# alpha-davidson/TensorBNN

Measured on AMD Instinct MI355X. Metric: leapfrog steps/sec (whole node), higher is better.
Workload: dtype f32

## Files before the change

tensorbnn_amd/csrc/fused_ops.hpp:

```cpp
#pragma once
#include <hip/hip_runtime.h>
#include "common.hpp"
#include "wide_api.hpp"

#define TBNN_JIT_ABI 7
enum { TBNN_FAMILY_NARROW = 1, TBNN_FAMILY_WIDE = 2 };

struct FusedOps {
    int abi;
    int family;
    int nl, dims[TBNN_MAX_LAYERS + 1];
    int hact, lact, lik;
    char name[128];
    int img_floats;
    void (*image_map)(int* map );
    int (*grid)(long n);
    int (*launch)(int grid, hipStream_t st, const NetDev* nd, const float* qimg, const float* eta, const float* X,
                  const float* Y, long n, float* slabs, int pitch, double* pstat, int nchains, ChainStride cs);
    int (*nforward)(int gx, int nets, hipStream_t st, const float* qimgs, long img_stride, const float* X, long n, float* fouts,
                    long out_stride);
    int traj_max_rows;
    int (*traj)(int nchains, hipStream_t st, const NetDev* nd, const float* qimg, long img_stride, const float* eta, const float* X, const float* Y, long n,
                float* q, float* p, float* g, float* gd, const int* imgmap, double* pstat, int nstat, float eps, int L, const StepCtl* ctl);
    void (*plan)(long n, WidePlan* plan);
    int (*wlaunch)(const WidePlan* plan, hipStream_t st, const NetDev* nd, const float* qimg, const float* eta,
                   const float* X, const float* Y, long n, float* store, float* slabA, float* slabB, double* pstat, float* out);
    int (*wforward)(hipStream_t st, const NetDev* nd, const float* qimg, const float* X, long n, float* fout);
};

static inline bool fused_ops_match(const FusedOps& o, const NetDev& nd, bool weighted = false) {
    if (o.nl != nd.nl || o.lik != (shape_lik(nd.lik) | (weighted ? SHAPE_LIK_WEIGHTED : 0))) return false;
    for (int l = 0; l < nd.nl; ++l) {
        if (nd.in[l] != o.dims[l] || nd.out[l] != o.dims[l + 1]) return false;
        if (nd.act[l] != (l == nd.nl - 1 ? o.lact : ((o.hact & TBNN_ACT_PACKED) ? (o.hact >> (3 * l)) & 7 : o.hact))) return false;
    }
    return true;
}

template <class S>
static inline void fused_ops_shape(FusedOps* o, const char* prefix, const char* name = nullptr) {
    o->abi = TBNN_JIT_ABI;
    o->nl = S::NL;
    for (int i = 0; i <= S::NL; ++i) o->dims[i] = S::D[i];
    o->hact = S::HCODE; o->lact = S::LACT; o->lik = S::LIK;
    if (name) { snprintf(o->name, sizeof(o->name), "%s", name); return; }
    static const char* an[] = {"none", "relu", "tanh", "sigmoid", "exp", "elu", "?", "?"};
    int k = snprintf(o->name, sizeof(o->name), "%s<", prefix);
    if (S::HCODE & TBNN_ACT_PACKED) {
// ... 7 lines not shown
```

tensorbnn_amd/csrc/jit_mid.hpp:

```cpp
#pragma once
#include "kernels_mid.hpp"
#include "fused_ops.hpp"

template <class S>
struct JitMid {
    static int grid(long n) { return mid_grid(n); }
    static int launch(int g, hipStream_t st, const NetDev* nd, const float* qimg, const float* eta, const float* X, const float* Y,
                      long n, float* slabs, int pitch, double* pstat, int nchains, ChainStride cs) {
        return mid_launch_t<S>(g, st, *nd, qimg, eta, X, Y, n, slabs, pitch, pstat, nchains, cs);
    }
    static int nforward(int gx, int nets, hipStream_t st, const float* qimgs, long img_stride, const float* X, long n, float* fouts,
                        long out_stride) {
        return mid_forward_t<S>(gx, nets, st, qimgs, img_stride, X, n, fouts, out_stride);
    }
    static void image_map(int* map) { mid_image_map<S>(map); }
    static void fill(FusedOps* o, const char* name = nullptr) {
        fused_ops_shape<S>(o, "jit-mid", name);
        o->family = TBNN_FAMILY_NARROW;
        o->img_floats = MidCfg<S>::IMG_FLOATS;
        o->image_map = &image_map; o->grid = &grid; o->launch = &launch; o->nforward = &nforward;
        o->plan = nullptr; o->wlaunch = nullptr; o->wforward = nullptr;
    }
};
```

tensorbnn_amd/csrc/jit_narrow.hpp:

```cpp
#pragma once
#include "kernels_fast3.hpp"
#include "kernels_traj.hpp"
#include "fused_ops.hpp"

template <class S, bool F3>
struct JitNarrow {
    static int grid(long n) {
        const long ntiles = (n + 15) / 16, wgs = (ntiles + FAST_WAVES - 1) / FAST_WAVES;
        return (int)(wgs < 256 ? wgs : 256);
    }
    static int launch_stamped(int g, hipStream_t st, const NetDev* nd, const float* qimg, const float* eta, const float* X, const float* Y,
                              long n, float* slabs, int pitch, double* pstat, int nchains, ChainStride cs, unsigned long long* stamps) {
        if constexpr (F3)
            hipLaunchKernelGGL(k_fwd_bwd_fast3<S>, dim3(g, nchains), dim3(FAST_THREADS), 0, st, *nd, qimg, eta, X, Y, n, slabs, pitch, pstat,
                               stamps, cs);
        else
            hipLaunchKernelGGL(k_fwd_bwd_fast<S>, dim3(g, nchains), dim3(FAST_THREADS), 0, st, *nd, qimg, eta, X, Y, n, slabs, pitch, pstat,
                               stamps, cs);
        return hipGetLastError() == hipSuccess ? 0 : -1;
    }
    static int launch(int g, hipStream_t st, const NetDev* nd, const float* qimg, const float* eta, const float* X, const float* Y,
                      long n, float* slabs, int pitch, double* pstat, int nchains, ChainStride cs) {
        return launch_stamped(g, st, nd, qimg, eta, X, Y, n, slabs, pitch, pstat, nchains, cs, nullptr);
    }
    static int nforward(int gx, int nets, hipStream_t st, const float* qimgs, long img_stride, const float* X, long n, float* fouts,
                        long out_stride) {
        if constexpr (F3) {
            hipLaunchKernelGGL(k_forward_fast3<S>, dim3(gx, nets), dim3(FAST_THREADS), 0, st, qimgs, img_stride, X, n, fouts, out_stride);
            return hipGetLastError() == hipSuccess ? 0 : -1;
        } else {
            return -1;
        }
    }
    static constexpr int TRAJ_NW = (!F3 || S::WTD || TBNN_TRAJ_WAVES == 0) ? 0 : (TBNN_TRAJ_WAVES == 16 && TrajCfg<S, 16>::OK) ? 16 : (TrajCfg<S, 4>::OK ? 4 : 0);
    static int traj(int nchains, hipStream_t st, const NetDev* nd, const float* qimg, long img_stride, const float* eta, const float* X, const float* Y, long n,
                    float* q, float* p, float* g, float* gd, const int* imgmap, double* pstat, int nstat, float eps, int L, const StepCtl* ctl) {
        if constexpr (TRAJ_NW > 0) {
            hipLaunchKernelGGL((k_traj_fast3<S, TRAJ_NW>), dim3(1, nchains), dim3(64 * TRAJ_NW), 0, st, *nd, qimg, img_stride, eta, X, Y, n, q, p, g, gd, imgmap,
                               pstat, nstat, eps, L, ctl);
            return hipGetLastError() == hipSuccess ? 0 : -1;
        } else {
            return -1;
        }
    }
    static void image_map(int* map) { ImageMap<S, 0>::run(map); }
    static void fill(FusedOps* o, const char* name = nullptr) {
        fused_ops_shape<S>(o, F3 ? "jit-fast3" : "jit-fast", name);
        o->family = TBNN_FAMILY_NARROW;
        o->img_floats = FastCfg<S>::STATIC_FLOATS;
        o->image_map = &image_map; o->grid = &grid; o->launch = &launch;
        o->nforward = F3 ? &nforward : nullptr;
        o->plan = nullptr; o->wlaunch = nullptr; o->wforward = nullptr;
        o->traj = TRAJ_NW > 0 ? &traj : nullptr;
        o->traj_max_rows = TRAJ_NW == 16 ? TBNN_TRAJ_MAX_ROWS : TRAJ_NW == 4 ? TBNN_TRAJ_MAX_ROWS_4 : 0;
    }
};

#ifdef TBNN_TILE_STAMPS
extern "C" int tbnn_jit_tile_stamps(unsigned long long* out64) {
    return hipMemcpyFromSymbol(out64, HIP_SYMBOL(g_tile_stamps), 64 * sizeof(unsigned long long)) == hipSuccess ? 0 : -1;
}
#endif
```

tensorbnn_amd/csrc/jit_tall.hpp:

```cpp
#pragma once
#include "kernels_tall.hpp"
#include "fused_ops.hpp"

template <class S>
struct JitTall {
    static int grid(long n) { return tall_grid<S>(n); }
    static int launch(int g, hipStream_t st, const NetDev* nd, const float* qimg, const float* eta, const float* X, const float* Y,
                      long n, float* slabs, int pitch, double* pstat, int nchains, ChainStride cs) {
        return tall_launch_t<S>(g, st, *nd, qimg, eta, X, Y, n, slabs, pitch, pstat, nchains, cs);
    }
    static int nforward(int gx, int nets, hipStream_t st, const float* qimgs, long img_stride, const float* X, long n, float* fouts,
                        long out_stride) {
        return tall_forward_t<S>(gx, nets, st, qimgs, img_stride, X, n, fouts, out_stride);
    }
    static void image_map(int* map) { tall_image_map<S>(map); }
    static void fill(FusedOps* o, const char* prefix = "jit-tall") {
        fused_ops_shape<S>(o, prefix);
        o->family = TBNN_FAMILY_NARROW;
        o->img_floats = TallCfg<S, TallPick<S>::NW>::IMG_FLOATS;
        o->image_map = &image_map; o->grid = &grid; o->launch = &launch; o->nforward = &nforward;
        o->plan = nullptr; o->wlaunch = nullptr; o->wforward = nullptr;
    }
};
```

tensorbnn_amd/csrc/jit_wide.hpp:

```cpp
#pragma once
#include "wide_api.hpp"
#include "kernels_wide.hpp"
#include "fused_ops.hpp"

template <class S>
struct JitWide {
    static void plan(long n, WidePlan* p) { p->id = -2; wide_plan_t<S>(n, *p); }
    static int wlaunch(const WidePlan* p, hipStream_t st, const NetDev* nd, const float* qimg, const float* eta, const float* X,
                       const float* Y, long n, float* store, float* slabA, float* slabB, double* pstat, float* out) {
        return wide_launch_t<S>(*p, st, *nd, qimg, eta, X, Y, n, store, slabA, slabB, pstat, out);
    }
    static int wforward(hipStream_t st, const NetDev* nd, const float* qimg, const float* X, long n, float* fout) {
        return wide_forward_t<S>(st, *nd, qimg, X, n, fout);
    }
    static void image_map(int* map) { wide_image_map<S>(map); }
    static void fill(FusedOps* o, const char* name = nullptr) {
        fused_ops_shape<S>(o, WideCfg<S>::RESIDENT ? "jit-wide(resident)" : "jit-wide", name);
        o->family = TBNN_FAMILY_WIDE;
        o->img_floats = WideCfg<S>::IMG_FLOATS;
        o->image_map = &image_map; o->grid = nullptr; o->launch = nullptr;
        o->plan = &plan; o->wlaunch = &wlaunch;
        o->wforward = wide_forward_ok<S>() ? &wforward : nullptr;
        o->nforward = nullptr;
    }
};
```

tensorbnn_amd/csrc/kernels_fast3.hpp:

```cpp
#pragma once
#include <type_traits>
#include "kernels_fast.hpp"

template <int I, int N, class F>
__device__ __forceinline__ void sfor3(F&& f) {
    if constexpr (I < N) { f(std::integral_constant<int, I>{}); sfor3<I + 1, N>(f); }
}
template <class S>
struct F3Cfg : FastCfg<S> {
    using B = FastCfg<S>;
    static constexpr int NF(int l) { return (B::out(l) % 16 == 1 || B::out(l) % 16 == 2) ? B::out(l) % 16 : 0; }
    static constexpr int MTF(int l) { return NF(l) ? B::MT(l) - 1 : B::MT(l); }
    static constexpr int fslot(int l, int f) { return 16 * MTF(l) + 4 * f; }
    static constexpr int funit(int l, int f) { return 16 * MTF(l) + f; }
    static constexpr int NLM3 = MTF(B::NL - 1) == 0 ? B::NL - 1 : B::NL;
    static_assert(NLM3 == B::NLM, "fast3 expects the same MFMA/VALU split of the last layer as fast");
    static constexpr int dw_tiles_plain() { int o = 0; for (int m = 0; m < NLM3; ++m) o += MTF(m) * B::NT(m); return o; }
    static constexpr bool NCF(int l) {
        return dw_tiles_plain() <= 39 && l < NLM3 && B::NT(l) >= 2 && MTF(l) >= 1 && MTF(l) <= 4 && B::in(l) + 1 - 16 * (B::NT(l) - 1) <= 4;
    }
    static constexpr int NTF(int l) { return NCF(l) ? B::NT(l) - 1 : B::NT(l); }
    static constexpr int dwt3(int l) { return MTF(l) * NTF(l) + (NCF(l) ? 2 : 0); }
    static constexpr int dwoff3(int l) { int o = 0; for (int m = 0; m < l && m < NLM3; ++m) o += dwt3(m); return o; }
    static constexpr int dwfr3(int l) { return dwoff3(l) + MTF(l) * NTF(l); }
    static constexpr int DW3_TILES = dwoff3(B::NL);
    static constexpr int KIN(int l) { return l == 0 ? B::KS0 : 4 * B::MT(l - 1); }
    static constexpr bool FB(int l) { return NF(l) > 0 && MTF(l) > 0; }
    static constexpr int fpn(int l) { return NF(l) == 0 ? 0 : (FB(l) ? 2 * B::NT(l) : NF(l) * (KIN(l) + 1)); }
    static constexpr int fpoff(int l) { int o = 0; for (int m = 0; m < l; ++m) o += fpn(m); return o; }
    static constexpr int FP_REGS = fpoff(B::NL);
    static constexpr int maxNF() { int m = 0; for (int l = 0; l < B::NL; ++l) m = NF(l) > m ? NF(l) : m; return m; }
    static constexpr int EP3_WANT = DW3_TILES * FAST_WAVES * 256 <= 39936 ? DW3_TILES : (DW3_TILES < 16 ? DW3_TILES : 16);
    static constexpr int PR = 16 + TBNN_PPAD;
    static constexpr int aoff3(int l) { int o = 0; for (int m = 0; m < l && m < NLM3; ++m) o += 16 * B::NT(m) * PR; return o; }
    static constexpr int doff3 = aoff3(NLM3);
    static constexpr int fdoff3 = doff3 + 16 * B::maxMT() * PR;
    static constexpr int WAVE3_FLOATS = fdoff3 + 128;
    static constexpr int MIN3 = B::STATIC_FLOATS + FAST_WAVES * WAVE3_FLOATS;
    static constexpr int LDS3_A = MIN3 > EP3_WANT * FAST_WAVES * 256 ? MIN3 : EP3_WANT * FAST_WAVES * 256;
    static constexpr int LDS3_FLOATS = LDS3_A > FAST_WAVES * (FP_REGS > 0 ? FP_REGS : 1) * 64 ? LDS3_A : FAST_WAVES * FP_REGS * 64;
    static constexpr int EP3_TILES = LDS3_FLOATS / (FAST_WAVES * 256) < DW3_TILES ? LDS3_FLOATS / (FAST_WAVES * 256) : (DW3_TILES > 0 ? DW3_TILES : 1);
};

template <class S>
struct Tile3 {
    using C = F3Cfg<S>;
    f32x4 a[C::ACT_TILES];
    float af[C::NL][C::maxNF() > 0 ? C::maxNF() : 1];
    float x0[C::KS0];
};

#ifndef TBNN_F3_M4ACC
#define TBNN_F3_M4ACC 2
#endif
template <class S, int K>
__device__ __forceinline__ f32x4 fringe_partials(const float* __restrict__ prow, const f32x4* tiles) {
    using C = F3Cfg<S>;
    constexpr int KG = C::cdiv(K, 16), NA = KG < TBNN_F3_M4ACC ? KG : TBNN_F3_M4ACC;
    f32x4 acc[NA];
#pragma unroll
    for (int a = 0; a < NA; ++a) acc[a] = f32x4{0.f, 0.f, 0.f, 0.f};
#pragma unroll
    for (int kt = 0; kt < KG; ++kt) {
        const f32x4 w = load_ks(prow + 16 * kt, C::ksteps(K, kt));
#pragma unroll
        for (int s = 0; s < C::ksteps(K, kt); ++s) acc[kt % NA] = mfma4(w[s], tiles[kt][s], acc[kt % NA]);
    }
#pragma unroll
    for (int st = 1; st < NA; st *= 2)
#pragma unroll
        for (int a = 0; a + st < NA; a += 2 * st) acc[a] += acc[a + st];
    return acc[0];
}
template <class S, int l, bool IMG = true>
struct Fwd3 {
// ... 1205 lines not shown
#pragma unroll
        for (int t = 0; t < C::KS0; ++t) {
            const int u = 4 * t + g;
            xn[t] = (ok && u < d_in) ? X[row * d_in + u] : 0.f;
        }
#pragma unroll
        for (int o = 0; o < d_out; ++o) yn[o] = ok ? Y[row * d_out + o] : 0.f;
        wn = row_weight<S>(Y, n, row, ok);
    };
    long main_end = ntiles;
    int ncoop = 0;
    if constexpr (CO::ENABLED) {
        const long G = gridDim.x, rem = ntiles % W;
        if (rem > 0 && rem <= 2 * G) { main_end = ntiles - rem; ncoop = rem <= G ? 1 : 2; }
    }
    if constexpr ((TBNN_SKEL & 1) != 0) { main_end = 0; ncoop = 0; }
    float xc[2][C::KS0], yc[2][d_out], wc[2];
#pragma unroll
    for (int j = 0; j < 2; ++j) {
        const long ct = main_end + (long)j * gridDim.x + blockIdx.x;
        const long row = ct * 16 + i16;
        const bool ok = CO::ENABLED && j < ncoop && ct < ntiles && row < n;
#pragma unroll
        for (int t = 0; t < C::KS0; ++t) {
            const int u = 4 * t + g;
            xc[j][t] = (ok && u < d_in) ? X[row * d_in + u] : 0.f;
        }
#pragma unroll
        for (int o = 0; o < d_out; ++o) yc[j][o] = ok ? Y[row * d_out + o] : 0.f;
        wc[j] = row_weight<S>(Y, n, row, ok);
    }
    long tile = wg;
    fetch(tile);
    constexpr bool WTDMA = C::STATIC_FLOATS > C::WB_FLOATS;
    if constexpr (WTDMA) {
        constexpr int WT = C::STATIC_FLOATS - C::WB_FLOATS, NCHUNK = (WT + 255) / 256;
        static_assert(C::WB_FLOATS % 4 == 0 && WT % 4 == 0, "16-B pieces");
        for (int c = wave; c < NCHUNK; c += FAST_WAVES) {
            const int off = C::WB_FLOATS + c * 256;
            if (c * 256 + lane * 4 < WT) lds_dma16(qimg + off + lane * 4, lds + off);
        }
    }
    {
        constexpr int N4 = (WTDMA ? C::WB_FLOATS : C::STATIC_FLOATS) / 4, IT = (N4 + FAST_THREADS - 1) / FAST_THREADS;
        const float4* src = reinterpret_cast<const float4*>(qimg);
        float4* dst = reinterpret_cast<float4*>(lds);
        float4 v[IT];
#pragma unroll
        for (int k = 0; k < IT; ++k) { const int e = tid + k * FAST_THREADS; v[k] = e < N4 ? src[e] : make_float4(0.f, 0.f, 0.f, 0.f); }
        __builtin_amdgcn_sched_barrier(0);
        float4* z = reinterpret_cast<float4*>(wl);
        for (int e = lane; e < C::WAVE3_FLOATS / 4; e += 64) z[e] = make_float4(0.f, 0.f, 0.f, 0.f);
        __builtin_amdgcn_sched_barrier(0);
#pragma unroll
        for (int k = 0; k < IT; ++k) { const int e = tid + k * FAST_THREADS; if (e < N4) dst[e] = v[k]; }
    }
    __syncthreads();
    TB_STAMP(1); TSTAMPO(58);

    constexpr int NFd = C::maxNF() > 0 ? C::maxNF() : 1;
    f32x4 dW[C::DW3_TILES > 0 ? C::DW3_TILES : 1];
#pragma unroll
    for (int t = 0; t < C::DW3_TILES; ++t) dW[t] = f32x4{0.f, 0.f, 0.f, 0.f};
    float FP[C::FP_REGS > 0 ? C::FP_REGS : 1];
#pragma unroll
    for (int t = 0; t < C::FP_REGS; ++t) FP[t] = 0.f;
    const float sigma = lik_sigma(nd, eta);
    const float inv_var = 1.f / (sigma * sigma);
    double stat = 0.0;

    if (g == 0) wl[C::aoff3(0) + d_in * C::PR + i16] = 1.f;
#pragma unroll
    for (int l = 1; l < C::NLM3; ++l)
        if (C::in(l) % 16 == 0 && g == 0) wl[C::aoff3(l) + C::in(l) * C::PR + i16] = 1.f;
    typename Fwd3<S, 0>::Pre P0;
    Fwd3<S, 0>::pre_all(P0, lds, i16, g);
// ... 208 lines not shown
```

tensorbnn_amd/csrc/tbnn_api.hip:

```cpp
#include <hip/hip_runtime.h>
#include <rccl/rccl.h>
#include <dlfcn.h>
#include <cmath>
#include <cstdio>
#include <cstdlib>
#include <cstring>
#include <memory>
#include <new>
#include <string>
#include <utility>
#include <vector>

#include "common.hpp"
#include "kernels_generic.hpp"
#include "kernels_hmc.hpp"
#include "kernels_hyper.hpp"
#include "kernels_layered.hpp"
#include "kernels_ensemble.hpp"
#include "aot_ops.hpp"
#include <mutex>

static thread_local std::string g_err;
static int fail(int code, const std::string& msg) { g_err = msg; return code; }

// ... 154 lines not shown
    const FusedOps* o = narrow_find(nd);
    if (!o && mid_on) o = mid_find(nd);
    if (!o) o = wide_find(nd);
    if (!o && !env_off("TBNN_REGISTERED")) o = find_jit(nd);
    if (!o && !env_off("TBNN_TALL")) o = tall_find(nd);
    return o;
}
extern "C" int tbnn_register_kernel_lib(const char* path) {
    if (!path) return fail(-1, "null path");
    void* lib = dlopen(path, RTLD_NOW | RTLD_LOCAL);
    if (!lib) return fail(-6, std::string("dlopen: ") + dlerror());
    typedef int (*ops_fn)(FusedOps*);
    ops_fn fn = (ops_fn)dlsym(lib, "tbnn_jit_ops");
    if (!fn) { dlclose(lib); return fail(-6, std::string(path) + " does not export tbnn_jit_ops"); }
    FusedOps* o = new (std::nothrow) FusedOps();
    if (!o) return fail(-4, "out of host memory");
    memset(o, 0, sizeof(*o));
    if (fn(o) != 0 || o->abi != TBNN_JIT_ABI || (o->family != TBNN_FAMILY_NARROW && o->family != TBNN_FAMILY_WIDE)) {
        delete o; dlclose(lib);
        return fail(-6, std::string(path) + ": kernel table rejected (ABI mismatch?)");
    }
    std::lock_guard<std::mutex> lk(g_jit_mu);
    g_jit.push_back(o);
    return 0;
}
extern "C" int tbnn_fused_kernel_available(const tbnn_net_desc* desc) {
    NetDev nd;
    int rc = build_netdev(desc, nd);
    if (rc) return rc;
    const FusedOps* o = find_ops(nd, true);
    if (!o) return 0;
    if (o == find_jit(nd)) return 3;
    return o->family == TBNN_FAMILY_WIDE ? 2 : 1;
}

static void default_eta(const NetDev& nd, std::vector<float>& eta) {
    eta.assign(nd.H, 0.f);
    for (int l = 0; l < nd.nl; ++l) {
        if (nd.prior[l] == TBNN_PRIOR_CAUCHY) {
            eta[4 * l + 1] = sqrtf(0.5f); eta[4 * l + 3] = sqrtf(0.5f);
        } else {
            eta[4 * l + 1] = 1.f; eta[4 * l + 3] = 1.f;
        }
    }
    if (nd.lik == TBNN_LIK_GAUSSIAN) eta[nd.H - 1] = sqrtf(0.1f);
}

extern "C" int tbnn_destroy(tbnn_handle h) {
    if (!h) return 0;
    hipSetDevice(h->device);
    if (h->stream) hipStreamSynchronize(h->stream);
    delete h;
    return 0;
}

static int create_impl(const tbnn_net_desc* desc, int device, uint64_t seed, uint32_t chain_id, int n_chains, tbnn_handle* out);
extern "C" int tbnn_create(const tbnn_net_desc* desc, int device, uint64_t seed, uint32_t chain_id, tbnn_handle* out) {
    return create_impl(desc, device, seed, chain_id, 1, out);
}
extern "C" int tbnn_create_multi(const tbnn_net_desc* desc, int device, uint64_t seed, uint32_t chain_id, int32_t n_chains, tbnn_handle* out) {
    if (n_chains < 1 || n_chains > 1024) return fail(-1, "n_chains must be in [1, 1024]");
    {
        NetDev nd;
        int rc = build_netdev(desc, nd);
        if (rc) return rc;
        if ((long long)n_chains * (long long)nd.P > 0x7FFFFFFFLL) return fail(-1, "n_chains x parameter count exceeds 2^31 - 1");
// ... 358 lines not shown
    ONE_CHAIN(h, "tbnn_gather_samples");
    HIPCHK(hipSetDevice(h->device));
    const size_t per = (size_t)h->nd.P + h->nd.H, tot = per * c->world;
    if (!d_out) {
        HIPCHK(c->gbuf.grow(tot, tot));
        d_out = c->gbuf;
    }
    HIPCHK(hipMemcpyAsync(h->tmp, h->q_cur, (size_t)h->nd.P * sizeof(float), hipMemcpyDeviceToDevice, h->stream));
    HIPCHK(hipMemcpyAsync(h->tmp + h->nd.P, h->eta, (size_t)h->nd.H * sizeof(float), hipMemcpyDeviceToDevice, h->stream));
    NCCLCHK(g_rccl.AllGather(h->tmp, d_out, per, ncclFloat, c->comm, h->stream));
    if (host_out) HIPCHK(hipMemcpyAsync(host_out, d_out, tot * sizeof(float), hipMemcpyDeviceToHost, h->stream));
    HIPCHK(hipStreamSynchronize(h->stream));
    return 0;
}
extern "C" int tbnn_set_row_shard(tbnn_handle h, tbnn_comm_handle c, int64_t n_total) {
    NEED(h);
    ONE_CHAIN(h, "tbnn_set_row_shard");
    HIPCHK(hipSetDevice(h->device));
    HIPCHK(hipStreamSynchronize(h->stream));
    if (c && n_total < 1) return fail(-1, "n_total must be >= 1");
    if (c && h->dYw) return fail(-1, "tbnn_set_row_shard: the handle has row weights (tbnn_set_row_weights): weighted row sharding needs the weight sum of all ranks");
    h->shard = c; h->n_total = c ? (long)n_total : 0;
    h->cur_valid = false;
    return 0;
}
static inline double rows_total(const tbnn_ctx* h) { return h->dYw ? h->wsum : (double)(h->shard ? h->n_total : h->n); }
static inline const float* pass_Y(const tbnn_ctx* h) { return h->dYw ? h->dYw : h->dY; }
static inline const float* pass_w(const tbnn_ctx* h) { return h->dYw ? h->dYw + (size_t)h->n * h->nd.d_out : nullptr; }
static inline int stat_entries(const tbnn_ctx* h) { return h->shard ? 1 : h->grid; }
static inline const double* stat_ptr(const tbnn_ctx* h) { return h->shard ? h->pstat_red : h->pstat; }
static inline const float* grad_slabs(const tbnn_ctx* h) { return (h->shard && !is_wide(h)) ? h->grow : h->slabs; }
static inline int grad_nslab(const tbnn_ctx* h) { return h->shard ? 1 : h->nslab; }

static int launch_fwd_bwd(tbnn_ctx* h, const float* q, const float* eta, const StepCtl* ctl = nullptr, int t = 0) {
    const float* img = nullptr;
    const int C = h->C;
    const long imgS = h->img_floats, slabS = (long)h->nslab * h->pitch;
    if (h->imgmap) {
        if (q == h->q && h->q_img_valid) img = h->qimg;
        else {
            hipLaunchKernelGGL(k_make_image, dim3((h->nd.P + 255) / 256, C), dim3(256), 0, h->stream, h->nd.P, q, h->imgmap, h->qimg_cur, (long)h->nd.P, imgS);
            img = h->qimg_cur;
        }
    }
    hipEvent_t a = nullptr, b = nullptr;
    const bool prof = h->profile > 0 && (h->launch_no++ % h->profile) == 0;
    if (prof) {
        if (h->pev_used + 2 > h->pev.size()) {
            hipEventCreate(&a); hipEventCreate(&b); h->pev.emplace_back(a); h->pev.emplace_back(b);
        }
        a = h->pev[h->pev_used]; b = h->pev[h->pev_used + 1]; h->pev_used += 2;
        h->pev_div.push_back(1);
        hipEventRecord(a, h->stream);
    }
    const ChainStride cs = {imgS, (long)h->nd.H, slabS, ctl, t};
    auto done = [&](int c) { return ctl != nullptr && t > h->ctl_host[c].L; };
    if (h->lay) {
        for (int c = 0; c < C; ++c)
            if (!done(c) && lay_launch(h->nd, h->lplan, h->stream, img + c * imgS, eta + (size_t)c * h->nd.H, pass_Y(h), h->n, h->lstore, h->slabs + c * slabS, h->pitch,
                           h->pstat + (size_t)c * PSTAT_CAP, pass_w(h)))
                return fail(-2, "layered kernel launch failed");
    } else if (is_wide(h)) {
        for (int c = 0; c < C; ++c) {
            if (done(c)) continue;
            const float* ic = img + c * imgS; const float* ec = eta + (size_t)c * h->nd.H;
            double* pc = h->pstat + (size_t)c * PSTAT_CAP; float* sl = h->slabs + c * slabS;
            if (h->ops->wlaunch(&h->wplan, h->stream, &h->nd, ic, ec, h->dX, pass_Y(h), h->n, h->wstore, h->wslabA, h->wslabB, pc, sl))
                return fail(-2, h->kernel_name + ": launch failed");
        }
    } else if (h->ops) {
        if (h->ops->launch(h->grid, h->stream, &h->nd, img, eta, h->dX, pass_Y(h), h->n, h->slabs, h->pitch, h->pstat, C, cs))
            return fail(-2, h->kernel_name + ": launch failed");
    } else {
        for (int c = 0; c < C; ++c)
            if (!done(c)) hipLaunchKernelGGL(k_fwd_bwd_generic, dim3(h->grid), dim3(GEN_RB), 0, h->stream, h->nd, q + (size_t)c * h->nd.P, eta + (size_t)c * h->nd.H, h->dX,
                               pass_Y(h), h->n, h->scratch, h->scratchPerWG, h->slabs + c * slabS, h->pitch, h->pstat + (size_t)c * PSTAT_CAP, pass_w(h));
    }
    if (h->shard) {
        float* row = is_wide(h) ? h->slabs : h->grow;
        const int P = h->nd.P;
        if (!is_wide(h))
            hipLaunchKernelGGL(k_slab_reduce, dim3((P + 63) / 64), dim3(64, 4), 0, h->stream, (const float*)h->slabs, h->nslab,
                               h->pitch, P, (float*)nullptr, h->shard_buf);
        hipLaunchKernelGGL(k_shard_pack, dim3((P + 255) / 256), dim3(256), 0, h->stream, P, is_wide(h) ? (const float*)row : (const float*)nullptr,
                           (const double*)h->pstat, h->grid, h->shard_buf);
        NCCLCHK(g_rccl.AllReduce(h->shard_buf, h->shard_buf, (size_t)P + 1, ncclDouble, ncclSum, h->shard->comm, h->stream));
        hipLaunchKernelGGL(k_shard_unpack, dim3((P + 255) / 256), dim3(256), 0, h->stream, P, (const double*)h->shard_buf, row, h->pstat_red);
    }
    if (prof) hipEventRecord(b, h->stream);
    HIPCHK(hipGetLastError());
    return 0;
}
static void launch_update(tbnn_ctx* h, int mode, float eps, const float* eta, float* q, float* g, const StepCtl* ctl = nullptr, int t = 0) {
    const bool big = h->nd.P >= UPD_BIG_P;
    const int ucols = big ? UPD_COLS_BIG : UPD_COLS;
    const int gx = (h->pitch / 4 + ucols - 1) / ucols;
    const bool img = h->imgmap && q == h->q;
    float* gd = g == h->g_cur ? h->gd_cur : (g == h->g ? h->gd : nullptr);
    if (big)
        hipLaunchKernelGGL((k_update<UPD_COLS_BIG, UPD_GROUPS_BIG>), dim3(gx, h->C), dim3(UPD_COLS_BIG, UPD_GROUPS_BIG), 0, h->stream, h->nd, mode, eps, eta,
                           grad_slabs(h), grad_nslab(h), h->pitch, h->q_cur, h->g_cur, q, h->p, g, img ? h->imgmap : nullptr, h->qimg, gd, h->img_floats, ctl, t);
    else
        hipLaunchKernelGGL((k_update<UPD_COLS, UPD_GROUPS>), dim3(gx, h->C), dim3(UPD_COLS, UPD_GROUPS), 0, h->stream, h->nd, mode, eps, eta, grad_slabs(h),
                           grad_nslab(h), h->pitch, h->q_cur, h->g_cur, q, h->p, g, img ? h->imgmap : nullptr, h->qimg, gd, h->img_floats, ctl, t);
    if (img && (mode == UPD_FIRST || mode == UPD_MID)) h->q_img_valid = true;
}
static void launch_energy(tbnn_ctx* h, int which, const float* eta, const float* q, double* slot) {
    hipLaunchKernelGGL(k_energy, dim3(1, h->C), dim3(1024), 0, h->stream, h->nd, which, eta, q, h->p, h->q_cur, stat_ptr(h),
                       stat_entries(h), rows_total(h), h->sc, slot);
}

static int ensure_current(tbnn_ctx* h, double* slot) {
    if (h->cur_valid) return 0;
    int rc = launch_fwd_bwd(h, h->q_cur, h->eta);
    if (rc) return rc;
    launch_update(h, UPD_GRAD_ONLY, 0.f, h->eta, h->q_cur, h->g_cur);
    launch_energy(h, EN_CUR, h->eta, h->q_cur, slot);
    h->cur_valid = true;
    return 0;
}
static float drain_profile(tbnn_ctx* h) {
    double tot = 0.0; int cnt = 0;
    for (size_t i = 0; i + 1 < h->pev_used; i += 2) {
        float ms = 0.f;
        const int div = i / 2 < h->pev_div.size() ? h->pev_div[i / 2] : 1;
        if (hipEventElapsedTime(&ms, h->pev[i], h->pev[i + 1]) == hipSuccess) { tot += ms * 1000.0 / (div > 0 ? div : 1); ++cnt; }
    }
    h->pev_used = 0;
    h->pev_div.clear();
    return cnt ? (float)(tot / cnt) : 0.f;
// ... 376 lines not shown
extern "C" int tbnn_metrics(tbnn_handle h, int which, const float* theta, float mean, float sd, int exp_pred, int exp_real,
                            double out3[3]) {
    NEED(h);
    if (!out3) return fail(-1, "null out3");
    if (which != 0 && which != 1) return fail(-1, "which must be 0 (training rows) or 1 (validation rows)");
    HIPCHK(hipSetDevice(h->device));
    long n = 0;
    int rc = predict_resident(h, which, theta, &n);
    if (rc) return rc;
    const int MB = 256;
    HIPCHK(h->mpart.grow(3 * MB, 3 * MB));
    const long tot = n * h->nd.d_out;
    const int grid = (int)std::min<long>(MB, (tot + 255) / 256);
    hipLaunchKernelGGL(k_metrics, dim3(grid), dim3(256), 0, h->stream, (const float*)h->fbuf, (const float*)(which ? h->dYv : h->dY), n,
                       h->nd.d_out, mean, sd, exp_pred, exp_real, h->mpart);
    HIPCHK(hipGetLastError());
    std::vector<double> part(3 * (size_t)grid);
    HIPCHK(hipMemcpyAsync(part.data(), h->mpart, part.size() * sizeof(double), hipMemcpyDeviceToHost, h->stream));
    HIPCHK(hipStreamSynchronize(h->stream));
    double a[3] = {0, 0, 0};
    for (int b = 0; b < grid; ++b) for (int k = 0; k < 3; ++k) a[k] += part[3 * b + k];
    for (int k = 0; k < 3; ++k) out3[k] = a[k] / (double)tot;
    return 0;
}

static int enqueue_transition(tbnn_ctx* h, float eps, int L, const float* d_p0, const float* d_logu, double* d_trace,
                              Scal* d_out, const StepCtl* ctl = nullptr) {
    const NetDev& nd = h->nd;
    const bool cached = h->cur_valid;
    int rc = ensure_current(h, d_trace);
    if (rc) return rc;
    if (d_trace && cached) hipLaunchKernelGGL(k_trace_logp_cur, dim3(1), dim3(64), 0, h->stream, (const Scal*)h->sc, d_trace);
    hipLaunchKernelGGL(k_begin, dim3(1, h->C), dim3(1024), 0, h->stream, nd, d_p0, d_logu, h->epoch, h->key0, h->key1, h->p, h->sc, h->seed_hi);
    launch_update(h, UPD_FIRST, eps, h->eta, h->q, h->g, ctl, 0);
    const bool traj = h->traj && !d_trace && L >= 1 && h->ops && h->ops->family == TBNN_FAMILY_NARROW && h->ops->traj && h->n <= h->ops->traj_max_rows &&
                      !h->shard;
    h->last_path = traj ? "trajectory" : "per-step";
    if (traj) {
        hipEvent_t ea = nullptr, eb = nullptr;
        const bool prof = h->profile > 0 && (h->launch_no++ % h->profile) == 0;
        if (prof) {
            if (h->pev_used + 2 > h->pev.size()) { hipEventCreate(&ea); hipEventCreate(&eb); h->pev.emplace_back(ea); h->pev.emplace_back(eb); }
            ea = h->pev[h->pev_used]; eb = h->pev[h->pev_used + 1]; h->pev_used += 2;
            h->pev_div.push_back(L);
            hipEventRecord(ea, h->stream);
        }
        const int trc = h->ops->traj(h->C, h->stream, &nd, h->qimg, (long)h->img_floats, h->eta, h->dX, h->dY, h->n, h->q, h->p, h->g, h->gd, h->imgmap,
                                     h->pstat, stat_entries(h), eps, L, ctl);
        if (prof) hipEventRecord(eb, h->stream);
        if (trc)
            return fail(-2, "trajectory kernel launch failed");
        h->q_img_valid = false;
    }
    for (int t = 1; t <= L && !traj; ++t) {
        rc = launch_fwd_bwd(h, h->q, h->eta, ctl, t);
        if (rc) return rc;
        if (d_trace && t < L) {
            launch_update(h, UPD_GRAD_ONLY, 0.f, h->eta, h->q, h->g);
            launch_energy(h, EN_TRACE, h->eta, h->q, d_trace + t);
        }
        launch_update(h, t < L ? UPD_MID : UPD_LAST, eps, h->eta, h->q, h->g, ctl, t);
    }
    if (h->merge_ends && nd.P <= 32768) {
        hipLaunchKernelGGL(k_energy, dim3(1, h->C), dim3(1024), 0, h->stream, h->nd, (int)EN_NEW, (const float*)h->eta, (const float*)h->q, (const float*)h->p,
                           (const float*)h->q_cur, stat_ptr(h), stat_entries(h), rows_total(h), h->sc, d_trace ? d_trace + L : (double*)nullptr,
                           d_out, (const float*)h->g, h->q_cur, h->g_cur, (const float*)h->gd, h->gd_cur);
    } else {
        launch_energy(h, EN_NEW, h->eta, h->q, d_trace ? d_trace + L : nullptr);
        hipLaunchKernelGGL(k_commit, dim3((nd.P + 255) / 256, h->C), dim3(256), 0, h->stream, nd.P, (const Scal*)h->sc, (const float*)h->q, (const float*)h->g,
// ... 245 lines not shown
    NEED(h); if (!p_out) return fail(-1, "null p_out");
    ONE_CHAIN(h, "tbnn_debug_momentum");
    HIPCHK(hipSetDevice(h->device));
    HIPCHK(hipMemcpyAsync(p_out, h->p, (size_t)h->nd.P * sizeof(float), hipMemcpyDeviceToHost, h->stream));
    HIPCHK(hipStreamSynchronize(h->stream));
    return 0;
}

extern "C" int tbnn_debug_draw(tbnn_handle h, uint32_t epoch, uint32_t purpose, int32_t n, float* out_normals,
                               float* out_log_u) {
    NEED(h);
    if (n < 1 || !out_normals) return fail(-1, "debug_draw: bad arguments");
    HIPCHK(hipSetDevice(h->device));
    Buf<float> d;
    HIPCHK(d.alloc((size_t)n + 1));
    hipLaunchKernelGGL(k_debug_draw, dim3((n + 255) / 256), dim3(256), 0, h->stream, epoch, purpose, h->key0, h->key1, (int)n, d, d + n);
    HIPCHK(hipGetLastError());
    std::vector<float> host(n + 1);
    HIPCHK(hipMemcpyAsync(host.data(), d, (size_t)(n + 1) * sizeof(float), hipMemcpyDeviceToHost, h->stream));
    HIPCHK(hipStreamSynchronize(h->stream));
    memcpy(out_normals, host.data(), (size_t)n * sizeof(float));
    if (out_log_u) *out_log_u = host[n];
    return 0;
}

extern "C" int tbnn_debug_stamps(tbnn_handle h, uint64_t* out5) {
    if (!out5) return fail(-1, "null out16");
    NEED(h);
    if (!h->ops || h->ops != narrow_find(h->nd) || !h->dX || h->C > 1) return fail(-1, "debug_stamps: narrow fast kernel + data required");
    HIPCHK(hipSetDevice(h->device));
    Buf<unsigned long long> d;
    HIPCHK(d.alloc(16));
    HIPCHK(hipMemset(d, 0, 16 * sizeof(unsigned long long)));
    hipLaunchKernelGGL(k_make_image, dim3((h->nd.P + 255) / 256), dim3(256), 0, h->stream, h->nd.P, h->q_cur, h->imgmap, h->qimg_cur);
    for (int rep = 0; rep < 3; ++rep)
        if (narrow_launch_stamped(h->ops, h->grid, h->stream, h->nd, h->qimg_cur, h->eta, h->dX, h->dY, h->n, h->slabs, h->pitch, h->pstat, d))
            return fail(-2, "debug_stamps: launch failed");
    HIPCHK(hipStreamSynchronize(h->stream));
    HIPCHK(hipMemcpy(out5, d, 16 * sizeof(uint64_t), hipMemcpyDeviceToHost));
    return 0;
}

extern "C" int tbnn_debug_fused_burst(tbnn_handle h, int32_t reps, float* us_per_pass) {
    if (!us_per_pass || reps < 1) return fail(-1, "fused_burst: reps >= 1 and an output pointer required");
    NEED(h);
    if (!h->dX) return fail(-1, "fused_burst: no data");
    if (h->shard) return fail(-1, "fused_burst: not on a row-sharded handle (every pass would be a collective; the other ranks are not in this call)");
    HIPCHK(hipSetDevice(h->device));
    const size_t PB = (size_t)h->C * h->nd.P * sizeof(float);
    HIPCHK(hipMemcpyAsync(h->q, h->q_cur, PB, hipMemcpyDeviceToDevice, h->stream));
    if (h->imgmap) {
        hipLaunchKernelGGL(k_make_image, dim3((h->nd.P + 255) / 256, h->C), dim3(256), 0, h->stream, h->nd.P, (const float*)h->q, h->imgmap, h->qimg, (long)h->nd.P,
                           (long)h->img_floats);
        h->q_img_valid = true;
    }
    struct ProfileOff {
        tbnn_ctx* h; int saved;
        explicit ProfileOff(tbnn_ctx* h_) : h(h_), saved(h_->profile) { h->profile = 0; }
        ~ProfileOff() { h->profile = saved; h->q_img_valid = false; }
    } guard(h);
    int rc = launch_fwd_bwd(h, h->q, h->eta);
    HIPCHK(hipEventRecord(h->ev0, h->stream));
    for (int r = 0; r < reps && !rc; ++r) rc = launch_fwd_bwd(h, h->q, h->eta);
    HIPCHK(hipEventRecord(h->ev1, h->stream));
    if (rc) return rc;
    HIPCHK(hipEventSynchronize(h->ev1));
    float ms = 0.f;
    HIPCHK(hipEventElapsedTime(&ms, h->ev0, h->ev1));
    *us_per_pass = ms * 1000.f / (float)reps;
// ... 16 lines not shown
```

Measured before the change: 20980.

## Build fast3 weight image in LDS directly from flat theta vector

For fast3 narrow kernels with at least 1024 parameters, each workgroup now loads the raw parameter vector q into LDS staging and scatters it into the padded and transposed weight image itself. This skips the separate k_make_image pass, and the update kernel's image write, on the per-step path. The cost is a per-workgroup scatter and extra LDS zeroing plus barriers inside the fused kernel. The trajectory path still asks for the image to be built.

```diff
diff --git a/tensorbnn_amd/csrc/fused_ops.hpp b/tensorbnn_amd/csrc/fused_ops.hpp
--- a/tensorbnn_amd/csrc/fused_ops.hpp
+++ b/tensorbnn_amd/csrc/fused_ops.hpp
@@ -3,7 +3,7 @@
 #include "common.hpp"
 #include "wide_api.hpp"
 
-#define TBNN_JIT_ABI 7
+#define TBNN_JIT_ABI 8
 enum { TBNN_FAMILY_NARROW = 1, TBNN_FAMILY_WIDE = 2 };
 
 struct FusedOps {
@@ -14,6 +14,7 @@
     char name[128];
     int img_floats;
     void (*image_map)(int* map );
+    void (*theta_slots)(int* map );
     int (*grid)(long n);
     int (*launch)(int grid, hipStream_t st, const NetDev* nd, const float* qimg, const float* eta, const float* X,
                   const float* Y, long n, float* slabs, int pitch, double* pstat, int nchains, ChainStride cs);
diff --git a/tensorbnn_amd/csrc/jit_mid.hpp b/tensorbnn_amd/csrc/jit_mid.hpp
--- a/tensorbnn_amd/csrc/jit_mid.hpp
+++ b/tensorbnn_amd/csrc/jit_mid.hpp
@@ -18,7 +18,7 @@
         fused_ops_shape<S>(o, "jit-mid", name);
         o->family = TBNN_FAMILY_NARROW;
         o->img_floats = MidCfg<S>::IMG_FLOATS;
-        o->image_map = &image_map; o->grid = &grid; o->launch = &launch; o->nforward = &nforward;
+        o->image_map = &image_map; o->theta_slots = nullptr; o->grid = &grid; o->launch = &launch; o->nforward = &nforward;
         o->plan = nullptr; o->wlaunch = nullptr; o->wforward = nullptr;
     }
 };
diff --git a/tensorbnn_amd/csrc/jit_narrow.hpp b/tensorbnn_amd/csrc/jit_narrow.hpp
--- a/tensorbnn_amd/csrc/jit_narrow.hpp
+++ b/tensorbnn_amd/csrc/jit_narrow.hpp
@@ -44,11 +44,14 @@
         }
     }
     static void image_map(int* map) { ImageMap<S, 0>::run(map); }
+    static constexpr bool THETA = F3 && F3Cfg<S>::FROM_THETA;
+    static void theta_slots(int* map) { if constexpr (THETA) theta_slot_map<S>(map); }
     static void fill(FusedOps* o, const char* name = nullptr) {
         fused_ops_shape<S>(o, F3 ? "jit-fast3" : "jit-fast", name);
         o->family = TBNN_FAMILY_NARROW;
         o->img_floats = FastCfg<S>::STATIC_FLOATS;
         o->image_map = &image_map; o->grid = &grid; o->launch = &launch;
+        o->theta_slots = THETA ? &theta_slots : nullptr;
         o->nforward = F3 ? &nforward : nullptr;
         o->plan = nullptr; o->wlaunch = nullptr; o->wforward = nullptr;
         o->traj = TRAJ_NW > 0 ? &traj : nullptr;
diff --git a/tensorbnn_amd/csrc/jit_tall.hpp b/tensorbnn_amd/csrc/jit_tall.hpp
--- a/tensorbnn_amd/csrc/jit_tall.hpp
+++ b/tensorbnn_amd/csrc/jit_tall.hpp
@@ -18,7 +18,7 @@
         fused_ops_shape<S>(o, prefix);
         o->family = TBNN_FAMILY_NARROW;
         o->img_floats = TallCfg<S, TallPick<S>::NW>::IMG_FLOATS;
-        o->image_map = &image_map; o->grid = &grid; o->launch = &launch; o->nforward = &nforward;
+        o->image_map = &image_map; o->theta_slots = nullptr; o->grid = &grid; o->launch = &launch; o->nforward = &nforward;
         o->plan = nullptr; o->wlaunch = nullptr; o->wforward = nullptr;
     }
 };
diff --git a/tensorbnn_amd/csrc/jit_wide.hpp b/tensorbnn_amd/csrc/jit_wide.hpp
--- a/tensorbnn_amd/csrc/jit_wide.hpp
+++ b/tensorbnn_amd/csrc/jit_wide.hpp
@@ -18,7 +18,7 @@
         fused_ops_shape<S>(o, WideCfg<S>::RESIDENT ? "jit-wide(resident)" : "jit-wide", name);
         o->family = TBNN_FAMILY_WIDE;
         o->img_floats = WideCfg<S>::IMG_FLOATS;
-        o->image_map = &image_map; o->grid = nullptr; o->launch = nullptr;
+        o->image_map = &image_map; o->theta_slots = nullptr; o->grid = nullptr; o->launch = nullptr;
         o->plan = &plan; o->wlaunch = &wlaunch;
         o->wforward = wide_forward_ok<S>() ? &wforward : nullptr;
         o->nforward = nullptr;
diff --git a/tensorbnn_amd/csrc/kernels_fast3.hpp b/tensorbnn_amd/csrc/kernels_fast3.hpp
--- a/tensorbnn_amd/csrc/kernels_fast3.hpp
+++ b/tensorbnn_amd/csrc/kernels_fast3.hpp
@@ -40,7 +40,52 @@
     static constexpr int LDS3_A = MIN3 > EP3_WANT * FAST_WAVES * 256 ? MIN3 : EP3_WANT * FAST_WAVES * 256;
     static constexpr int LDS3_FLOATS = LDS3_A > FAST_WAVES * (FP_REGS > 0 ? FP_REGS : 1) * 64 ? LDS3_A : FAST_WAVES * FP_REGS * 64;
     static constexpr int EP3_TILES = LDS3_FLOATS / (FAST_WAVES * 256) < DW3_TILES ? LDS3_FLOATS / (FAST_WAVES * 256) : (DW3_TILES > 0 ? DW3_TILES : 1);
+    static constexpr int STG_FLOATS = (B::P() + 3 + 3) / 4 * 4;
+    static constexpr bool FROM_THETA = B::P() >= 1024 && STG_FLOATS <= FAST_WAVES * WAVE3_FLOATS;
 };
+
+template <class S, int l, int WV, class F>
+__host__ __device__ __forceinline__ void theta_row_slots(int i, F&& f) {
+    using C = F3Cfg<S>;
+    constexpr int in = C::in(l), out = C::out(l);
+    constexpr bool WT = l >= 1 && l < C::NLM;
+    const int ri = slot_of(out, i);
+    const int src = C::offW(l) + i * in, w = C::woff(l) + ri * C::LDW(l), t = C::toff(l) + ri;
+#pragma unroll
+    for (int k = WV; k < in; k += 4) {
+        const int ck = l == 0 ? k : slot_of(in, k);
+        f(src + k, w + ck, WT ? t + ck * C::LDT(l) : -1);
+    }
+    if (in % 4 == WV) f(C::offW(l) + in * out + i, C::boff(l) + ri, -1);
+}
+template <class S, int WV>
+struct ThetaImg {
+    using C = F3Cfg<S>;
+    static __device__ __forceinline__ void run(float* __restrict__ lds, const float* __restrict__ stg, int lane) {
+        sfor3<0, C::NL>([&](auto l_) __attribute__((always_inline)) {
+            constexpr int l = decltype(l_)::value;
+#pragma unroll
+            for (int r0 = 0; r0 < C::out(l); r0 += 64) {
+                const int i = r0 + lane;
+                if (i < C::out(l))
+                    theta_row_slots<S, l, WV>(i, [&](int j, int w, int t) __attribute__((always_inline)) {
+                        const float v = stg[j];
+                        lds[w] = v;
+                        if (t >= 0) lds[t] = v;
+                    });
+            }
+        });
+    }
+};
+template <class S, int l = 0, int WV = 0>
+static void theta_slot_map(int* map) {
+    using C = F3Cfg<S>;
+    if constexpr (l == 0 && WV == 0) for (int j = 0; j < 2 * C::P(); ++j) map[j] = -1;
+    for (int i = 0; i < C::out(l); ++i)
+        theta_row_slots<S, l, WV>(i, [&](int j, int w, int t) { map[j] = w; map[C::P() + j] = t; });
+    if constexpr (WV + 1 < 4) theta_slot_map<S, l, WV + 1>(map);
+    else if constexpr (l + 1 < C::NL) theta_slot_map<S, l + 1, 0>(map);
+}
 
 template <class S>
 struct Tile3 {
@@ -1312,7 +1357,7 @@
     }
     long tile = wg;
     fetch(tile);
-    constexpr bool WTDMA = C::STATIC_FLOATS > C::WB_FLOATS;
+    constexpr bool WTDMA = !C::FROM_THETA && C::STATIC_FLOATS > C::WB_FLOATS;
     if constexpr (WTDMA) {
         constexpr int WT = C::STATIC_FLOATS - C::WB_FLOATS, NCHUNK = (WT + 255) / 256;
         static_assert(C::WB_FLOATS % 4 == 0 && WT % 4 == 0, "16-B pieces");
@@ -1321,7 +1366,42 @@
             if (c * 256 + lane * 4 < WT) lds_dma16(qimg + off + lane * 4, lds + off);
         }
     }
-    {
+    if constexpr (C::FROM_THETA) {
+        constexpr int P = C::P(), SN = C::STG_FLOATS, IT = (SN / 4 + FAST_THREADS - 1) / FAST_THREADS;
+        const int sh = (int)((reinterpret_cast<size_t>(qimg) >> 2) & 3);
+        const float* base = qimg - sh;
+        float* stg = lds + C::STATIC_FLOATS;
+        float4 v[IT];
+#pragma unroll
+        for (int k = 0; k < IT; ++k) {
+            const int lo = 4 * (tid + k * FAST_THREADS), end = sh + P;
+            if (lo + 3 < end) v[k] = *reinterpret_cast<const float4*>(base + lo);
+            else {
+                v[k] = make_float4(0.f, 0.f, 0.f, 0.f);
+                if (lo < end) v[k].x = base[lo];
+                if (lo + 1 < end) v[k].y = base[lo + 1];
+                if (lo + 2 < end) v[k].z = base[lo + 2];
+            }
+        }
+        __builtin_amdgcn_sched_barrier(0);
+        float4* z = reinterpret_cast<float4*>(lds);
+        constexpr int Z0 = C::STATIC_FLOATS / 4, Z1 = (C::STATIC_FLOATS + SN) / 4, Z2 = (C::STATIC_FLOATS + FAST_WAVES * C::WAVE3_FLOATS) / 4;
+        static_assert(C::STATIC_FLOATS % 4 == 0 && C::WAVE3_FLOATS % 4 == 0, "16-B pieces");
+        for (int e = tid; e < Z0; e += FAST_THREADS) z[e] = make_float4(0.f, 0.f, 0.f, 0.f);
+        for (int e = Z1 + tid; e < Z2; e += FAST_THREADS) z[e] = make_float4(0.f, 0.f, 0.f, 0.f);
+        __builtin_amdgcn_sched_barrier(0);
+#pragma unroll
+        for (int k = 0; k < IT; ++k) { const int e = tid + k * FAST_THREADS; if (e < SN / 4) reinterpret_cast<float4*>(stg)[e] = v[k]; }
+        __syncthreads();
+        switch (wave) {
+            case 0: ThetaImg<S, 0>::run(lds, stg + sh, lane); break;
+            case 1: ThetaImg<S, 1>::run(lds, stg + sh, lane); break;
+            case 2: ThetaImg<S, 2>::run(lds, stg + sh, lane); break;
+            default: ThetaImg<S, 3>::run(lds, stg + sh, lane); break;
+        }
+        __syncthreads();
+        for (int e = Z0 + tid; e < Z1; e += FAST_THREADS) z[e] = make_float4(0.f, 0.f, 0.f, 0.f);
+    } else {
         constexpr int N4 = (WTDMA ? C::WB_FLOATS : C::STATIC_FLOATS) / 4, IT = (N4 + FAST_THREADS - 1) / FAST_THREADS;
         const float4* src = reinterpret_cast<const float4*>(qimg);
         float4* dst = reinterpret_cast<float4*>(lds);
diff --git a/tensorbnn_amd/csrc/tbnn_api.hip b/tensorbnn_amd/csrc/tbnn_api.hip
--- a/tensorbnn_amd/csrc/tbnn_api.hip
+++ b/tensorbnn_amd/csrc/tbnn_api.hip
@@ -210,6 +210,19 @@
     if (!o) return 0;
     if (o == find_jit(nd)) return 3;
     return o->family == TBNN_FAMILY_WIDE ? 2 : 1;
+}
+
+extern "C" int tbnn_debug_image_slots(const tbnn_net_desc* desc, int32_t* image_map, int32_t* theta_slots, int32_t* img_floats) {
+    NetDev nd;
+    int rc = build_netdev(desc, nd);
+    if (rc) return rc;
+    const FusedOps* o = find_ops(nd, true);
+    if (img_floats) *img_floats = o ? o->img_floats : 0;
+    if (!o) return 0;
+    if (image_map) o->image_map(image_map);
+    if (!o->theta_slots) return 0;
+    if (theta_slots) o->theta_slots(theta_slots);
+    return 1;
 }
 
 static void default_eta(const NetDev& nd, std::vector<float>& eta) {
@@ -634,11 +647,13 @@
 static inline const float* grad_slabs(const tbnn_ctx* h) { return (h->shard && !is_wide(h)) ? h->grow : h->slabs; }
 static inline int grad_nslab(const tbnn_ctx* h) { return h->shard ? 1 : h->nslab; }
 
+static inline bool theta_direct(const tbnn_ctx* h) { return h->ops && h->ops->theta_slots; }
 static int launch_fwd_bwd(tbnn_ctx* h, const float* q, const float* eta, const StepCtl* ctl = nullptr, int t = 0) {
     const float* img = nullptr;
     const int C = h->C;
-    const long imgS = h->img_floats, slabS = (long)h->nslab * h->pitch;
-    if (h->imgmap) {
+    const long imgS = theta_direct(h) ? (long)h->nd.P : (long)h->img_floats, slabS = (long)h->nslab * h->pitch;
+    if (theta_direct(h)) img = q;
+    else if (h->imgmap) {
         if (q == h->q && h->q_img_valid) img = h->qimg;
         else {
             hipLaunchKernelGGL(k_make_image, dim3((h->nd.P + 255) / 256, C), dim3(256), 0, h->stream, h->nd.P, q, h->imgmap, h->qimg_cur, (long)h->nd.P, imgS);
@@ -693,11 +708,12 @@
     HIPCHK(hipGetLastError());
     return 0;
 }
-static void launch_update(tbnn_ctx* h, int mode, float eps, const float* eta, float* q, float* g, const StepCtl* ctl = nullptr, int t = 0) {
+static void launch_update(tbnn_ctx* h, int mode, float eps, const float* eta, float* q, float* g, const StepCtl* ctl = nullptr, int t = 0,
+                          bool want_image = false) {
     const bool big = h->nd.P >= UPD_BIG_P;
     const int ucols = big ? UPD_COLS_BIG : UPD_COLS;
     const int gx = (h->pitch / 4 + ucols - 1) / ucols;
-    const bool img = h->imgmap && q == h->q;
+    const bool img = h->imgmap && q == h->q && (want_image || !theta_direct(h));
     float* gd = g == h->g_cur ? h->gd_cur : (g == h->g ? h->gd : nullptr);
     if (big)
         hipLaunchKernelGGL((k_update<UPD_COLS_BIG, UPD_GROUPS_BIG>), dim3(gx, h->C), dim3(UPD_COLS_BIG, UPD_GROUPS_BIG), 0, h->stream, h->nd, mode, eps, eta,
@@ -1140,9 +1156,9 @@
     if (rc) return rc;
     if (d_trace && cached) hipLaunchKernelGGL(k_trace_logp_cur, dim3(1), dim3(64), 0, h->stream, (const Scal*)h->sc, d_trace);
     hipLaunchKernelGGL(k_begin, dim3(1, h->C), dim3(1024), 0, h->stream, nd, d_p0, d_logu, h->epoch, h->key0, h->key1, h->p, h->sc, h->seed_hi);
-    launch_update(h, UPD_FIRST, eps, h->eta, h->q, h->g, ctl, 0);
     const bool traj = h->traj && !d_trace && L >= 1 && h->ops && h->ops->family == TBNN_FAMILY_NARROW && h->ops->traj && h->n <= h->ops->traj_max_rows &&
                       !h->shard;
+    launch_update(h, UPD_FIRST, eps, h->eta, h->q, h->g, ctl, 0, traj);
     h->last_path = traj ? "trajectory" : "per-step";
     if (traj) {
         hipEvent_t ea = nullptr, eb = nullptr;
@@ -1454,9 +1470,10 @@
     Buf<unsigned long long> d;
     HIPCHK(d.alloc(16));
     HIPCHK(hipMemset(d, 0, 16 * sizeof(unsigned long long)));
-    hipLaunchKernelGGL(k_make_image, dim3((h->nd.P + 255) / 256), dim3(256), 0, h->stream, h->nd.P, h->q_cur, h->imgmap, h->qimg_cur);
+    if (!theta_direct(h))
+        hipLaunchKernelGGL(k_make_image, dim3((h->nd.P + 255) / 256), dim3(256), 0, h->stream, h->nd.P, h->q_cur, h->imgmap, h->qimg_cur);
     for (int rep = 0; rep < 3; ++rep)
-        if (narrow_launch_stamped(h->ops, h->grid, h->stream, h->nd, h->qimg_cur, h->eta, h->dX, h->dY, h->n, h->slabs, h->pitch, h->pstat, d))
+        if (narrow_launch_stamped(h->ops, h->grid, h->stream, h->nd, theta_direct(h) ? (const float*)h->q_cur : (const float*)h->qimg_cur, h->eta, h->dX, h->dY, h->n, h->slabs, h->pitch, h->pstat, d))
             return fail(-2, "debug_stamps: launch failed");
     HIPCHK(hipStreamSynchronize(h->stream));
     HIPCHK(hipMemcpy(out5, d, 16 * sizeof(uint64_t), hipMemcpyDeviceToHost));
```

Result: slower. 20450 (-2.5%).
